# mryab/learning-at-home

Hardware: NVIDIA H100
Metric: DMoE training samples/sec (whole job, device-timed, max over ranks) (higher is better)
Workload: dtype bf16

## Files before the change

learning-at-home_b200/csrc/layernorm.cu:

```cuda
#include "sm90.cuh"
#include <cuda_fp8.h>
#include <stdlib.h>

#include <array>
#include <utility>

namespace lah {

constexpr float LN_EPS = 1e-5f;

constexpr int LN_MAX_C = 4096;

template <int C>
struct LnFwdCfg {
    static constexpr int NV = (C + 255) / 256;
    static constexpr bool TUNED = C >= 256 && (C & (C - 1)) == 0;
    static constexpr int R = TUNED ? ((NV * 4 <= 16) ? 4 : ((NV * 2 <= 16) ? 2 : 1)) : (NV <= 2 ? 4 : (NV <= 6 ? 2 : 1));
    static constexpr int MIN_BLOCKS = (TUNED || NV <= 12) ? 2 : 1;
};

static int ln_rows_per_warp(int dflt) {
    static int forced = -1;
    if (forced < 0) {
        const char* e = getenv("LAH_LN_ROWS");
        forced = e ? atoi(e) : 0;
    }
    return forced == 1 ? 1 : dflt;
}

template <int C, bool QUANT, int R>
__global__ void __launch_bounds__(256, LnFwdCfg<C>::MIN_BLOCKS) ln_relu_fwd_kernel(
    const bf16* __restrict__ h, bf16* __restrict__ a, float* __restrict__ mean_out, float* __restrict__ rstd_out,
    const float* __restrict__ gamma, const float* __restrict__ beta, const int* __restrict__ tile_group, int rows,
    int relu, uint8_t* __restrict__ aq, uint8_t* __restrict__ sf, int tile_shift) {
    constexpr int NV = LnFwdCfg<C>::NV;
    constexpr bool HALF = C % 256 != 0;
    static_assert(C % 128 == 0 && C <= LN_MAX_C && !(QUANT && HALF), "unsupported LayerNorm width");
    const int warp = threadIdx.x >> 5, lane = threadIdx.x & 31;
    const int row0 = (blockIdx.x * 8 + warp) * R;
    if (row0 >= rows) return;
    const int g = tile_group ? __ldg(tile_group + (row0 >> tile_shift)) : 0;
    if (g < 0) return;
    int4 q[R][NV];
#pragma unroll
    for (int r = 0; r < R; ++r) {
        const int4* hp = reinterpret_cast<const int4*>(h + static_cast<long long>(min(row0 + r, rows - 1)) * C);
#pragma unroll
        for (int j = 0; j < NV; ++j) {
            if constexpr (HALF) {
                if (j == NV - 1 && lane >= 16) {
                    q[r][j] = make_int4(0, 0, 0, 0);
                    continue;
                }
            }
            q[r][j] = ld_nc_v4(hp + j * 32 + lane);
        }
    }
    float mean[R], rstd[R];
#pragma unroll
    for (int r = 0; r < R; ++r) {
        float s = 0.f, ss = 0.f;
#pragma unroll
        for (int j = 0; j < NV; ++j) {
            const uint32_t w[4] = {(uint32_t)q[r][j].x, (uint32_t)q[r][j].y, (uint32_t)q[r][j].z, (uint32_t)q[r][j].w};
#pragma unroll
            for (int t = 0; t < 4; ++t) {
                const float2 f = unpack_bf16x2(w[t]);
                s += f.x + f.y;
                ss += f.x * f.x + f.y * f.y;
            }
        }
        s = warp_sum(s);
        ss = warp_sum(ss);
        mean[r] = s * (1.f / C);
        rstd[r] = rsqrtf(fmaxf(ss * (1.f / C) - mean[r] * mean[r], 0.f) + LN_EPS);
        if (lane == 0 && mean_out && row0 + r < rows) {
            mean_out[row0 + r] = mean[r];
            rstd_out[row0 + r] = rstd[r];
        }
    }
    const float* gp = gamma + static_cast<long long>(g) * C;
    const float* bp = beta + static_cast<long long>(g) * C;
#pragma unroll
    for (int j = 0; j < NV; ++j) {
        if constexpr (HALF) {
            if (j == NV - 1 && lane >= 16) break;
        }
        const int col = (j * 32 + lane) * 8;
        const int4 g0 = ld_nc_v4(reinterpret_cast<const int4*>(gp + col));
        const int4 g1 = ld_nc_v4(reinterpret_cast<const int4*>(gp + col + 4));
        const int4 b0 = ld_nc_v4(reinterpret_cast<const int4*>(bp + col));
        const int4 b1 = ld_nc_v4(reinterpret_cast<const int4*>(bp + col + 4));
        const float gg[8] = {__int_as_float(g0.x), __int_as_float(g0.y), __int_as_float(g0.z), __int_as_float(g0.w),
                             __int_as_float(g1.x), __int_as_float(g1.y), __int_as_float(g1.z), __int_as_float(g1.w)};
        const float bb[8] = {__int_as_float(b0.x), __int_as_float(b0.y), __int_as_float(b0.z), __int_as_float(b0.w),
                             __int_as_float(b1.x), __int_as_float(b1.y), __int_as_float(b1.z), __int_as_float(b1.w)};
#pragma unroll
        for (int r = 0; r < R; ++r) {
            const int row = row0 + r;
            if (row >= rows) continue;
            const uint32_t w[4] = {(uint32_t)q[r][j].x, (uint32_t)q[r][j].y, (uint32_t)q[r][j].z, (uint32_t)q[r][j].w};
            float y[8];
#pragma unroll
            for (int t = 0; t < 4; ++t) {
                const float2 f = unpack_bf16x2(w[t]);
                y[2 * t] = (f.x - mean[r]) * rstd[r] * gg[2 * t] + bb[2 * t];
                y[2 * t + 1] = (f.y - mean[r]) * rstd[r] * gg[2 * t + 1] + bb[2 * t + 1];
            }
            if (relu) {
#pragma unroll
                for (int t = 0; t < 8; ++t) y[t] = fmaxf(y[t], 0.f);
            }
            if (!QUANT || a) {
                int4 o;
                o.x = pack_bf16x2(y[0], y[1]);
                o.y = pack_bf16x2(y[2], y[3]);
                o.z = pack_bf16x2(y[4], y[5]);
                o.w = pack_bf16x2(y[6], y[7]);
                st_v4(reinterpret_cast<int4*>(a + static_cast<long long>(row) * C) + j * 32 + lane, o);
            }
            if (QUANT) {
                float amax = 0.f;
#pragma unroll
                for (int t = 0; t < 8; ++t) amax = fmaxf(amax, fabsf(y[t]));
                amax = fmaxf(amax, __shfl_xor_sync(0xffffffffu, amax, 1));
                amax = fmaxf(amax, __shfl_xor_sync(0xffffffffu, amax, 2));
                const uint32_t bits = __float_as_uint(amax * (1.f / 448.f));
                uint32_t e = ((bits >> 23) & 0xFFu) + ((bits & 0x7FFFFFu) ? 1u : 0u);
                e = min(max(e, 1u), 253u);
                const float inv = __uint_as_float((254u - e) << 23);
                uint2 o8;
                o8.x = static_cast<uint32_t>(__nv_cvt_float2_to_fp8x2(make_float2(y[0] * inv, y[1] * inv), __NV_SATFINITE, __NV_E4M3)) |
                       (static_cast<uint32_t>(__nv_cvt_float2_to_fp8x2(make_float2(y[2] * inv, y[3] * inv), __NV_SATFINITE, __NV_E4M3)) << 16);
                o8.y = static_cast<uint32_t>(__nv_cvt_float2_to_fp8x2(make_float2(y[4] * inv, y[5] * inv), __NV_SATFINITE, __NV_E4M3)) |
                       (static_cast<uint32_t>(__nv_cvt_float2_to_fp8x2(make_float2(y[6] * inv, y[7] * inv), __NV_SATFINITE, __NV_E4M3)) << 16);
                asm volatile("st.global.v2.u32 [%0], {%1, %2};" ::"l"(reinterpret_cast<uint2*>(aq + static_cast<long long>(row) * C) + j * 32 + lane),
                             "r"(o8.x), "r"(o8.y)
                             : "memory");
                if ((lane & 3) == 0) {
                    const int kb32 = j * 8 + (lane >> 2);
                    const int ra = row & 127;
                    const long long chunk = static_cast<long long>(row >> 7) * (C / 128) + (kb32 >> 2);
                    sf[chunk * 512 + ((ra & 31) * 4 + (ra >> 5)) * 4 + (kb32 & 3)] = static_cast<uint8_t>(e);
                }
            }
        }
    }
}

template <int C>
struct LnBwdCfg {
    static constexpr int THREADS = (C / 8 + 31) / 32 * 32;
    static constexpr int MIN_BLOCKS = (C <= 2048) ? 2 : 1;
    static constexpr int RB = ((THREADS / 32 * MIN_BLOCKS + 3) / 4 >= 4 && C != 2048) ? 2 : 4;
};

template <int C, bool RES>
__global__ void __launch_bounds__(LnBwdCfg<C>::THREADS, LnBwdCfg<C>::MIN_BLOCKS) ln_relu_bwd_kernel(const bf16* __restrict__ da, const bf16* __restrict__ h,
                                                            const float* __restrict__ mean_in,
                                                            const float* __restrict__ rstd_in,
                                                            const float* __restrict__ gamma,
                                                            const float* __restrict__ beta, bf16* __restrict__ dh,
                                                            float* __restrict__ part,
                                                            const int* __restrict__ tile_group, int rows, int relu, int tile_rows,
                                                            const bf16* __restrict__ dres) {
    constexpr int THREADS = LnBwdCfg<C>::THREADS;
    constexpr int WARPS = THREADS / 32;
    constexpr bool IDLE = THREADS * 8 != C;
    static_assert(C % 128 == 0 && C <= LN_MAX_C, "unsupported LayerNorm width");
    constexpr int RB = LnBwdCfg<C>::RB;
    __shared__ float red[WARPS][2 * RB];
    __shared__ float tot[2 * RB];
    const int tile = blockIdx.x;
    const int g = tile_group ? __ldg(tile_group + tile) : 0;
    if (g < 0) return;
    const int tid = threadIdx.x, warp = tid >> 5, lane = tid & 31;
    const int col = tid * 8;
    const bool live = !IDLE || col < C;
    float gam[8], bet[8];
    if (!live) {
#pragma unroll
        for (int t = 0; t < 8; ++t) gam[t] = bet[t] = 0.f;
    } else {
        const float* gp = gamma + static_cast<long long>(g) * C + col;
        const float* bp = beta + static_cast<long long>(g) * C + col;
        const float4 g0 = __ldg(reinterpret_cast<const float4*>(gp)), g1 = __ldg(reinterpret_cast<const float4*>(gp + 4));
        const float4 b0 = __ldg(reinterpret_cast<const float4*>(bp)), b1 = __ldg(reinterpret_cast<const float4*>(bp + 4));
        gam[0] = g0.x; gam[1] = g0.y; gam[2] = g0.z; gam[3] = g0.w; gam[4] = g1.x; gam[5] = g1.y; gam[6] = g1.z; gam[7] = g1.w;
        bet[0] = b0.x; bet[1] = b0.y; bet[2] = b0.z; bet[3] = b0.w; bet[4] = b1.x; bet[5] = b1.y; bet[6] = b1.z; bet[7] = b1.w;
    }
    float acc_dg[8], acc_db[8], acc_dbias[8];
#pragma unroll
    for (int t = 0; t < 8; ++t) acc_dg[t] = acc_db[t] = acc_dbias[t] = 0.f;

    const int row0 = tile * tile_rows;
    const int row_end = min(rows, row0 + tile_rows);
    int4 nqa[RB], nqh[RB];
    float nmu[RB], nrs[RB];
    auto issue_loads = [&](int rb) {
#pragma unroll
        for (int r = 0; r < RB; ++r) {
            const int row = rb + r;
            const int rr = row < row_end ? row : row0;
            const long long off = static_cast<long long>(rr) * C + col;
            if (live) {
                nqa[r] = ld_nc_v4(reinterpret_cast<const int4*>(da + off));
                nqh[r] = ld_nc_v4(reinterpret_cast<const int4*>(h + off));
            } else {
                nqa[r] = nqh[r] = make_int4(0, 0, 0, 0);
            }
            nmu[r] = __ldg(mean_in + rr);
            nrs[r] = __ldg(rstd_in + rr);
        }
    };
    issue_loads(row0);
    for (int rb = row0; rb < row_end; rb += RB) {
        float rs[RB];
        float part[2 * RB];
        int4 qa_c[RB], qh_c[RB];
        float mu_c[RB];
#pragma unroll
        for (int r = 0; r < RB; ++r) {
            qa_c[r] = nqa[r];
            qh_c[r] = nqh[r];
            mu_c[r] = nmu[r];
            rs[r] = nrs[r];
        }
        if (rb + RB < row_end) issue_loads(rb + RB);
        auto slice = [&](int r, bool ok, float (&gvv)[8], float (&xhh)[8]) {
            const uint32_t wa[4] = {(uint32_t)qa_c[r].x, (uint32_t)qa_c[r].y, (uint32_t)qa_c[r].z, (uint32_t)qa_c[r].w};
            const uint32_t wh[4] = {(uint32_t)qh_c[r].x, (uint32_t)qh_c[r].y, (uint32_t)qh_c[r].z, (uint32_t)qh_c[r].w};
#pragma unroll
            for (int t = 0; t < 4; ++t) {
                const float2 fa = unpack_bf16x2(wa[t]);
                const float2 fh = unpack_bf16x2(wh[t]);
                const float x0 = (fh.x - mu_c[r]) * rs[r], x1 = (fh.y - mu_c[r]) * rs[r];
                const float y0 = x0 * gam[2 * t] + bet[2 * t], y1 = x1 * gam[2 * t + 1] + bet[2 * t + 1];
                gvv[2 * t] = (ok && (!relu || y0 > 0.f)) ? fa.x : 0.f;
                gvv[2 * t + 1] = (ok && (!relu || y1 > 0.f)) ? fa.y : 0.f;
                xhh[2 * t] = x0;
                xhh[2 * t + 1] = x1;
            }
        };
#pragma unroll
        for (int r = 0; r < RB; ++r) {
            float gvv[8], xhh[8];
            slice(r, rb + r < row_end, gvv, xhh);
            float s1 = 0.f, s2 = 0.f;
#pragma unroll
            for (int t = 0; t < 8; ++t) {
                const float d = gvv[t] * gam[t];
                s1 += d;
                s2 += d * xhh[t];
            }
            part[2 * r] = s1;
            part[2 * r + 1] = s2;
        }
#pragma unroll
        for (int i = 0; i < 2 * RB; ++i) part[i] = warp_sum(part[i]);
        if (lane == 0) {
#pragma unroll
            for (int i = 0; i < 2 * RB; ++i) red[warp][i] = part[i];
        }
        __syncthreads();
        if (tid < 2 * RB) {
            float s = 0.f;
#pragma unroll
            for (int w = 0; w < WARPS; ++w) s += red[w][tid];
            tot[tid] = s * (1.f / C);
        }
        __syncthreads();
#pragma unroll
        for (int r = 0; r < RB; ++r) {
            const int row = rb + r;
            if (row >= row_end || !live) continue;
            float gvv[8], xhh[8];
            slice(r, true, gvv, xhh);
            const float m1 = tot[2 * r], m2 = tot[2 * r + 1];
            float o[8], res[8];
            if (RES) {
                const int4 qr = ld_nc_v4(reinterpret_cast<const int4*>(dres + static_cast<long long>(row) * C + col));
                const uint32_t wr[4] = {(uint32_t)qr.x, (uint32_t)qr.y, (uint32_t)qr.z, (uint32_t)qr.w};
#pragma unroll
                for (int t = 0; t < 4; ++t) {
                    const float2 fr = unpack_bf16x2(wr[t]);
                    res[2 * t] = fr.x;
                    res[2 * t + 1] = fr.y;
                }
            }
#pragma unroll
            for (int t = 0; t < 8; ++t) {
                o[t] = rs[r] * (gvv[t] * gam[t] - m1 - xhh[t] * m2);
                if (RES) o[t] += res[t];
                acc_db[t] += gvv[t];
                acc_dg[t] += gvv[t] * xhh[t];
                acc_dbias[t] += o[t];
            }
            int4 q;
            q.x = pack_bf16x2(o[0], o[1]);
            q.y = pack_bf16x2(o[2], o[3]);
            q.z = pack_bf16x2(o[4], o[5]);
            q.w = pack_bf16x2(o[6], o[7]);
            *reinterpret_cast<int4*>(dh + static_cast<long long>(row) * C + col) = q;
        }
    }
    if (!live) return;
    float* pg = part + static_cast<long long>(tile) * 3 * C + col;
#pragma unroll
    for (int t = 0; t < 8; ++t) {
        pg[t] = acc_dg[t];
        pg[C + t] = acc_db[t];
        pg[2 * C + t] = acc_dbias[t];
    }
}

__global__ void __launch_bounds__(512) grouped_colsum_kernel(const bf16* __restrict__ x, long long ldx,
                                                             float* __restrict__ part, int C,
                                                             const int* __restrict__ tile_group, int rows, int tile_rows) {
    __shared__ float2 sm[4][128];
    const int tile = blockIdx.x;
    const int g = tile_group ? __ldg(tile_group + tile) : 0;
    if (g < 0) return;
    const int cp = threadIdx.x & 127;
    const int phase = threadIdx.x >> 7;
    const int col = blockIdx.y * 256 + cp * 2;
    if (col >= C) return;
    const int row0 = tile * tile_rows, row_end = min(rows, row0 + tile_rows);
    float2 acc = make_float2(0.f, 0.f);
    for (int r = row0 + phase; r < row_end; r += 4) {
        const uint32_t u = __ldg(reinterpret_cast<const uint32_t*>(x + static_cast<long long>(r) * ldx + col));
        const float2 f = unpack_bf16x2(u);
        acc.x += f.x;
        acc.y += f.y;
    }
    sm[phase][cp] = acc;
    __syncthreads();
    if (phase == 0) {
        float2 s = sm[0][cp];
#pragma unroll
        for (int p = 1; p < 4; ++p) {
            s.x += sm[p][cp].x;
            s.y += sm[p][cp].y;
        }
        *reinterpret_cast<float2*>(part + static_cast<long long>(tile) * C + col) = s;
    }
}

__global__ void __launch_bounds__(256) group_tile_sum_kernel(const float* __restrict__ part, int num_tiles, int V, int C,
                                                             const int* __restrict__ tile_group, float* out0, float* out1,
                                                             float* out2) {
    const int i = blockIdx.x * blockDim.x + threadIdx.x;
    if (i >= V * C) return;
    const int v = i / C, c = i - v * C;
    float* out = v == 0 ? out0 : (v == 1 ? out1 : out2);
    int cur = -1;
    float acc = 0.f;
    for (int t = 0; t < num_tiles; ++t) {
        const int g = tile_group ? __ldg(tile_group + t) : 0;
        if (g < 0) continue;
        if (g != cur) {
            if (cur >= 0) out[static_cast<long long>(cur) * C + c] += acc;
            cur = g;
            acc = 0.f;
        }
        acc += __ldg(part + (static_cast<long long>(t) * V + v) * C + c);
    }
    if (cur >= 0) out[static_cast<long long>(cur) * C + c] += acc;
}

using LnFwdLaunch = void (*)(const void*, void*, float*, float*, const float*, const float*, const int*, int, int, int,
                             cudaStream_t);
using LnBwdLaunch = void (*)(const void*, const void*, const float*, const float*, const float*, const float*, void*,
                             float*, float*, float*, float*, const int*, int, int, int, const void*, cudaStream_t);

template <int C>
void ln_fwd_launch(const void* h, void* a, float* mean, float* rstd, const float* gamma, const float* beta,
                   const int* tile_group, int rows, int relu, int tile_shift, cudaStream_t st) {
    constexpr int RR = LnFwdCfg<C>::R;
    if constexpr (LnFwdCfg<C>::TUNED) {
        if (ln_rows_per_warp(RR) == 1) {
            ln_relu_fwd_kernel<C, false, 1><<<(rows + 7) / 8, 256, 0, st>>>(
                (const bf16*)h, (bf16*)a, mean, rstd, gamma, beta, tile_group, rows, relu, nullptr, nullptr, tile_shift);
            return;
        }
    }
    ln_relu_fwd_kernel<C, false, RR><<<(rows + 8 * RR - 1) / (8 * RR), 256, 0, st>>>(
        (const bf16*)h, (bf16*)a, mean, rstd, gamma, beta, tile_group, rows, relu, nullptr, nullptr, tile_shift);
}

template <int C>
void ln_bwd_launch(const void* da, const void* h, const float* mean, const float* rstd, const float* gamma,
                   const float* beta, void* dh, float* dgamma, float* dbeta, float* dbias, float* part,
                   const int* tile_group, int rows, int relu, int tile_rows, const void* dres, cudaStream_t st) {
    const int grid = (rows + tile_rows - 1) / tile_rows;
    constexpr int T = LnBwdCfg<C>::THREADS;
    if (dres)
        ln_relu_bwd_kernel<C, true><<<grid, T, 0, st>>>((const bf16*)da, (const bf16*)h, mean, rstd, gamma, beta,
                                                        (bf16*)dh, part, tile_group, rows, relu, tile_rows,
                                                        (const bf16*)dres);
    else
        ln_relu_bwd_kernel<C, false><<<grid, T, 0, st>>>((const bf16*)da, (const bf16*)h, mean, rstd, gamma, beta,
                                                         (bf16*)dh, part, tile_group, rows, relu, tile_rows, nullptr);
    group_tile_sum_kernel<<<(3 * C + 255) / 256, 256, 0, st>>>(part, grid, 3, C, tile_group, dgamma, dbeta, dbias);
}

template <int... I>
constexpr auto ln_fwd_table(std::integer_sequence<int, I...>) {
    return std::array<LnFwdLaunch, sizeof...(I)>{ln_fwd_launch<(I + 1) * 128>...};
}
template <int... I>
constexpr auto ln_bwd_table(std::integer_sequence<int, I...>) {
    return std::array<LnBwdLaunch, sizeof...(I)>{ln_bwd_launch<(I + 1) * 128>...};
}
constexpr auto kLnFwd = ln_fwd_table(std::make_integer_sequence<int, LN_MAX_C / 128>{});
constexpr auto kLnBwd = ln_bwd_table(std::make_integer_sequence<int, LN_MAX_C / 128>{});

static bool ln_width_ok(int C) { return C > 0 && C % 128 == 0 && C <= LN_MAX_C; }

}

using namespace lah;

extern "C" {

static int shift_of(int tile_rows) {
    int s = 0;
    while ((1 << s) < tile_rows) ++s;
    return ((1 << s) == tile_rows && tile_rows >= 8) ? s : -1;
}

int lah_ln_relu_fwd(const void* h, void* a, float* mean, float* rstd, const float* gamma, const float* beta,
                    const int* tile_group, int rows, int C, int relu, int tile_rows, cudaStream_t st) {
    if (rows <= 0) return 0;
    const int tile_shift = shift_of(tile_rows);
    if (tile_shift < 0 || !ln_width_ok(C)) return -2;
    kLnFwd[C / 128 - 1](h, a, mean, rstd, gamma, beta, tile_group, rows, relu, tile_shift, st);
    return -(int)cudaGetLastError();
}

int lah_ln_relu_fwd_q(const void* h, void* a, float* mean, float* rstd, const float* gamma, const float* beta,
                      const int* tile_group, int rows, int C, int relu, void* aq, void* sf, cudaStream_t st) {
    if (rows <= 0) return 0;
#define LAH_LN_FWD(CC)                                                                                          \
    if (C == CC) {                                                                                              \
        constexpr int RR = LnFwdCfg<CC>::R;                                                                     \
        if (ln_rows_per_warp(RR) == 1)                                                                          \
            ln_relu_fwd_kernel<CC, true, 1><<<(rows + 7) / 8, 256, 0, st>>>(                                  \
                (const bf16*)h, (bf16*)a, mean, rstd, gamma, beta, tile_group, rows, relu, (uint8_t*)aq, (uint8_t*)sf, 7);   \
        else                                                                                                    \
            ln_relu_fwd_kernel<CC, true, RR><<<(rows + 8 * RR - 1) / (8 * RR), 256, 0, st>>>(                 \
                (const bf16*)h, (bf16*)a, mean, rstd, gamma, beta, tile_group, rows, relu, (uint8_t*)aq, (uint8_t*)sf, 7);   \
        return -(int)cudaGetLastError();                                                                        \
    }
    LAH_LN_FWD(256) LAH_LN_FWD(512) LAH_LN_FWD(1024) LAH_LN_FWD(2048) LAH_LN_FWD(4096)
#undef LAH_LN_FWD
    return -2;
}

int lah_ln_relu_bwd(const void* da, const void* h, const float* mean, const float* rstd, const float* gamma,
                    const float* beta, void* dh, float* dgamma, float* dbeta, float* dbias, float* part,
                    const int* tile_group, int rows, int C, int relu, int tile_rows, const void* dres, cudaStream_t st) {
    if (rows <= 0) return 0;
    if (shift_of(tile_rows) < 0 || !ln_width_ok(C)) return -2;
    kLnBwd[C / 128 - 1](da, h, mean, rstd, gamma, beta, dh, dgamma, dbeta, dbias, part, tile_group, rows, relu,
                        tile_rows, dres, st);
    return -(int)cudaGetLastError();
}

int lah_grouped_colsum(const void* x, long long ldx, float* out, float* part, int C, const int* tile_group, int rows,
                       int tile_rows, cudaStream_t st) {
    if (rows <= 0) return 0;
    if (C % 128 || shift_of(tile_rows) < 0) return -2;
    const int tiles = (rows + tile_rows - 1) / tile_rows;
    dim3 grid(tiles, (C + 255) / 256);
    grouped_colsum_kernel<<<grid, 512, 0, st>>>((const bf16*)x, ldx, part, C, tile_group, rows, tile_rows);
    group_tile_sum_kernel<<<(C + 255) / 256, 256, 0, st>>>(part, tiles, 1, C, tile_group, out, nullptr, nullptr);
    return -(int)cudaGetLastError();
}

}
```

learning-at-home_b200/csrc/small_m.cu:

```cuda
#include "sm90.cuh"
#include <climits>

namespace lah {
namespace smallm {

constexpr int BM = 128;
constexpr int BK = 64;
constexpr int MMA_K = 16;
constexpr int BN_MAX = 128;
constexpr int NUM_THREADS = 288;

namespace sab {

constexpr int STAGES = 6;
constexpr int A_BYTES = BM * BK * 2;
constexpr int B_BYTES = BN_MAX * BK * 2;
constexpr int STAGE_BYTES = A_BYTES + B_BYTES;
constexpr int BAR_OFFSET = STAGES * STAGE_BYTES;
constexpr int QD = 4;
constexpr int MAX_G = 1023;
constexpr int CUM_OFFSET = BAR_OFFSET + (2 * STAGES + 2 * QD) * 8 + QD * 4 + 16;
constexpr int SMEM_TOTAL = CUM_OFFSET + (MAX_G + 1) * 4 + 1024;
static_assert(SMEM_TOTAL <= 232448, "shared memory budget");

struct Params {
    int G, M_out, K;
    const int* group_off;
    const int* group_rows;
    bf16* out;
    long long ldo;
    const float* bias;
    const bf16* residual;
    long long ldr;
    const int* wait_flags;
    int wait_count, wait_epoch;
    const int* epoch_base;
    int* status;
    int* tile_counter;
};

__device__ __forceinline__ int box_rows_of(int nn) { return nn <= 16 ? 16 : (nn <= 32 ? 32 : (nn <= 64 ? 64 : 128)); }

__device__ __forceinline__ int find_group(const int* cum, int G, int gc) {
    int lo = 0, hi = G - 1;
    while (lo < hi) {
        const int mid = (lo + hi + 1) >> 1;
        if (cum[mid] <= gc) lo = mid; else hi = mid - 1;
    }
    return lo;
}

template <int NB, bool A_MN>
__device__ __forceinline__ void sab_tile(const Params& p, uint8_t* smem, uint64_t* full_bar, uint64_t* empty_bar, int& stage,
                                         uint32_t& phase, int num_kb, int wg, int warp, int lane, int g, int ms, int row0,
                                         int nn) {
    float acc[NB / 2];
    constexpr uint32_t A_KSTEP = A_MN ? MMA_K * 128 : MMA_K * 2;
    int prev_stage = -1;
    for (int kb = 0; kb < num_kb; ++kb) {
        mbar_wait(&full_bar[stage], phase);
        const uint32_t sa = smem_u32(smem + stage * STAGE_BYTES) + wg * (A_MN ? BK * 128 : 64 * 128);
        const uint32_t sb = smem_u32(smem + stage * STAGE_BYTES + A_BYTES);
        wgmma_fence();
#pragma unroll
        for (int k = 0; k < BK / MMA_K; ++k) {
            const uint64_t da = make_smem_desc_sw128(sa + k * A_KSTEP, BK * 128, 1024);
            const uint64_t db = make_smem_desc_sw128(sb + k * (MMA_K * 2), 0, 1024);
            const uint32_t accum = (kb > 0 || k > 0) ? 1u : 0u;
            if constexpr (NB == 16) wgmma_bf16_n16<A_MN, 0>(acc, da, db, accum);
            if constexpr (NB == 32) wgmma_bf16_n32<A_MN, 0>(acc, da, db, accum);
            if constexpr (NB == 64) wgmma_bf16_n64<A_MN, 0>(acc, da, db, accum);
            if constexpr (NB == 128) wgmma_bf16_n128<A_MN, 0>(acc, da, db, accum);
        }
        wgmma_commit();
        wgmma_wait<1>();
        if (prev_stage >= 0) {
            __syncwarp();
            if (lane == 0) mbar_arrive(&empty_bar[prev_stage]);
        }
        prev_stage = stage;
        if (++stage == STAGES) {
            stage = 0;
            phase ^= 1;
        }
    }
    wgmma_wait<0>();
    wgmma_fence_regs(acc);
    __syncwarp();
    if (lane == 0 && prev_stage >= 0) mbar_arrive(&empty_bar[prev_stage]);

    const int n16 = (nn + 15) & ~15;
#pragma unroll
    for (int h = 0; h < 2; ++h) {
        const int feat = ms * BM + wg * 64 + (warp & 3) * 16 + (lane >> 2) + 8 * h;
        const float bias = p.bias ? __ldg(p.bias + static_cast<long long>(g) * p.M_out + feat) : 0.f;
#pragma unroll
        for (int j = 0; j < NB / 8; ++j) {
#pragma unroll
            for (int e = 0; e < 2; ++e) {
                const int n = 8 * j + 2 * (lane & 3) + e;
                if (n < n16) {
                    const long long row = row0 + n;
                    float v = acc[4 * j + 2 * h + e] + bias;
                    if (p.residual) v += __bfloat162float(p.residual[row * p.ldr + feat]);
                    p.out[row * p.ldo + feat] = __float2bfloat16(v);
                }
            }
        }
    }
}

template <bool A_MN>
__global__ void __launch_bounds__(NUM_THREADS, 1)
swapab_kernel(const Params p, const __grid_constant__ CUtensorMap tmA, const __grid_constant__ CUtensorMap tmB16,
              const __grid_constant__ CUtensorMap tmB32, const __grid_constant__ CUtensorMap tmB64,
              const __grid_constant__ CUtensorMap tmB128) {
    extern __shared__ uint8_t smem_raw[];
    uint8_t* smem = reinterpret_cast<uint8_t*>((reinterpret_cast<uintptr_t>(smem_raw) + 1023) & ~uintptr_t(1023));
    uint64_t* full_bar = reinterpret_cast<uint64_t*>(smem + BAR_OFFSET);
    uint64_t* empty_bar = full_bar + STAGES;
    uint64_t* q_full = empty_bar + STAGES;
    uint64_t* q_empty = q_full + QD;
    volatile int* q_tile = reinterpret_cast<volatile int*>(q_empty + QD);
    int* cum = reinterpret_cast<int*>(smem + CUM_OFFSET);

    const int warp = threadIdx.x >> 5;
    const int lane = threadIdx.x & 31;

    if (warp == 0) {
        int carry = 0;
        for (int base = 0; base < p.G; base += 32) {
            const int g = base + lane;
            int x = g < p.G ? (__ldg(p.group_rows + g) + BN_MAX - 1) / BN_MAX : 0;
#pragma unroll
            for (int d = 1; d < 32; d <<= 1) {
                const int y = __shfl_up_sync(0xffffffffu, x, d);
                if (lane >= d) x += y;
            }
            if (g < p.G) cum[g + 1] = carry + x;
            carry += __shfl_sync(0xffffffffu, x, 31);
        }
        if (lane == 0) cum[0] = 0;
    }
    if (warp == 8 && lane == 0) {
        tma_prefetch_desc(&tmA);
        tma_prefetch_desc(&tmB16);
        tma_prefetch_desc(&tmB32);
        tma_prefetch_desc(&tmB64);
        tma_prefetch_desc(&tmB128);
        for (int i = 0; i < STAGES; ++i) {
            mbar_init(&full_bar[i], 1);
            mbar_init(&empty_bar[i], 8);
        }
        for (int i = 0; i < QD; ++i) {
            mbar_init(&q_full[i], 1);
            mbar_init(&q_empty[i], 8);
        }
        fence_mbar_init();
    }
    __syncthreads();

    const int m_slices = p.M_out / BM;
    const int total = cum[p.G] * m_slices;
    const int num_kb = p.K / BK;

    if (warp == 8) {
        if (lane != 0) return;
        if (p.wait_flags) {
            const int epoch = p.wait_epoch + (p.epoch_base ? *p.epoch_base : 0);
            const unsigned long long t_wait = globaltimer_ns();
            for (int sidx = 0; sidx < p.wait_count; ++sidx)
                spin_flag_ft(p.wait_flags + sidx, epoch, p.status, sidx, p.epoch_base ? p.epoch_base[1] : 0);
            if (blockIdx.x == 0) atomicAdd(reinterpret_cast<unsigned long long*>(p.status + 2), globaltimer_ns() - t_wait);
            fence_proxy_async_global();
        }
        int stage = 0, qi = 0;
        uint32_t phase = 0, qphase = 0;
        while (true) {
            const int tile = atomicAdd(p.tile_counter, 1);
            mbar_wait(&q_empty[qi], qphase ^ 1);
            q_tile[qi] = tile;
            mbar_arrive(&q_full[qi]);
            if (++qi == QD) {
                qi = 0;
                qphase ^= 1;
            }
            if (tile >= total) break;
            const int gc = tile / m_slices, ms = tile - gc * m_slices;
            const int g = find_group(cum, p.G, gc);
            const int n0 = (gc - cum[g]) * BN_MAX;
            const int rows = __ldg(p.group_rows + g);
            const int off = __ldg(p.group_off + g);
            const int box = box_rows_of(min(rows - n0, BN_MAX));
            const CUtensorMap* tmB = box == 16 ? &tmB16 : (box == 32 ? &tmB32 : (box == 64 ? &tmB64 : &tmB128));
            for (int kb = 0; kb < num_kb; ++kb) {
                mbar_wait(&empty_bar[stage], phase ^ 1);
                uint8_t* sa = smem + stage * STAGE_BYTES;
                uint8_t* sb = sa + A_BYTES;
                const int k = kb * BK;
                mbar_arrive_expect_tx(&full_bar[stage], A_BYTES + box * 128);
                if (!A_MN) {
                    tma_load_3d(sa, &tmA, &full_bar[stage], k, ms * BM, g);
                } else {
#pragma unroll
                    for (int i = 0; i < BM / 64; ++i)
                        tma_load_3d(sa + i * (BK * 128), &tmA, &full_bar[stage], ms * BM + i * 64, k, g);
                }
                tma_load_2d(sb, tmB, &full_bar[stage], k, off + n0);
                if (++stage == STAGES) {
                    stage = 0;
                    phase ^= 1;
                }
            }
        }
        return;
    }

    const int wg = warp >> 2;
    int stage = 0, qi = 0;
    uint32_t phase = 0, qphase = 0;
    while (true) {
        mbar_wait(&q_full[qi], qphase);
        const int tile = q_tile[qi];
        __syncwarp();
        if (lane == 0) mbar_arrive(&q_empty[qi]);
        if (++qi == QD) {
            qi = 0;
            qphase ^= 1;
        }
        if (tile >= total) break;
        const int gc = tile / m_slices, ms = tile - gc * m_slices;
        const int g = find_group(cum, p.G, gc);
        const int n0 = (gc - cum[g]) * BN_MAX;
        const int nn = min(__ldg(p.group_rows + g) - n0, BN_MAX);
        const int row0 = __ldg(p.group_off + g) + n0;
        switch (box_rows_of(nn)) {
            case 16: sab_tile<16, A_MN>(p, smem, full_bar, empty_bar, stage, phase, num_kb, wg, warp, lane, g, ms, row0, nn); break;
            case 32: sab_tile<32, A_MN>(p, smem, full_bar, empty_bar, stage, phase, num_kb, wg, warp, lane, g, ms, row0, nn); break;
            case 64: sab_tile<64, A_MN>(p, smem, full_bar, empty_bar, stage, phase, num_kb, wg, warp, lane, g, ms, row0, nn); break;
            default: sab_tile<128, A_MN>(p, smem, full_bar, empty_bar, stage, phase, num_kb, wg, warp, lane, g, ms, row0, nn); break;
        }
    }
}

}

namespace wa {

constexpr int WBK = 32;
constexpr int OP_STAGES = 2;
constexpr int OP_STAGE_BYTES = 2 * (WBK * BM * 2);
constexpr int OP_BYTES = OP_STAGES * OP_STAGE_BYTES;
constexpr int BAND_ROWS = 4;
constexpr int CHUNKS = 16 / BAND_ROWS;
constexpr int SUB_COLS = 32;
constexpr int SUB_BYTES = BM / CHUNKS * SUB_COLS * 4;
constexpr int ARR_BYTES = (BN_MAX / SUB_COLS) * SUB_BYTES;
constexpr int ST_STAGES = 3;
constexpr int ST_STAGE_BYTES = 4 * ARR_BYTES;
constexpr int ST_OFFSET = OP_BYTES;
constexpr int BAR_OFFSET = ST_OFFSET + ST_STAGES * ST_STAGE_BYTES;
constexpr int QD = 4;
constexpr int SMEM_TOTAL = BAR_OFFSET + (2 * OP_STAGES + 2 * ST_STAGES + 2 * QD) * 8 + QD * 4 + 16 + 1024;
static_assert(ST_STAGES <= CHUNKS, "the producer issues a tile's first ST_STAGES chunks before its remaining k-blocks");
static_assert(OP_STAGE_BYTES % 1024 == 0 && SUB_BYTES % 1024 == 0, "128-B swizzle atoms need 1 KB alignment");
static_assert(SMEM_TOTAL <= 232448, "shared memory budget");

struct Params {
    int G, N, K;
    const int* group_off;
    const int* group_rows;
    const int* skip;
    const int* step;
    float* p;
    float* m;
    float* v;
    float* vmax;
    bf16* p_bf16;
    float lr, beta1, beta2, eps;
    int amsgrad;
    float wd;
    int* tile_counter;
    const int* poison;
};

constexpr int WD_NONE = 0, WD_L2 = 1, WD_DECOUPLED = 2;

struct Tile {
    int g, mt, nt;
};

struct StateMaps {
    CUtensorMap a[4];
};

__device__ __forceinline__ void state_chunk_tma(const StateMaps& tm, int n_arr, uint8_t* ss, uint64_t* bar, int col0, int srow,
                                                int c) {
    for (int a = 0; a < n_arr; ++a)
#pragma unroll
        for (int q = 0; q < BN_MAX / SUB_COLS; ++q) {
            uint8_t* s = ss + a * ARR_BYTES + q * SUB_BYTES;
            if (bar) tma_load_3d(s, &tm.a[a], bar, col0 + q * SUB_COLS, BAND_ROWS * c, srow / 16);
            else tma_store_3d(&tm.a[a], s, col0 + q * SUB_COLS, BAND_ROWS * c, srow / 16);
        }
}

template <int WD>
__global__ void __launch_bounds__(NUM_THREADS, 1)
wgrad_adam_kernel(const Params p, const __grid_constant__ CUtensorMap tmDY, const __grid_constant__ CUtensorMap tmX,
                  const __grid_constant__ StateMaps tmS) {
    extern __shared__ uint8_t smem_raw[];
    uint8_t* smem = reinterpret_cast<uint8_t*>((reinterpret_cast<uintptr_t>(smem_raw) + 1023) & ~uintptr_t(1023));
    uint8_t* st_smem = smem + ST_OFFSET;
    uint64_t* op_full = reinterpret_cast<uint64_t*>(smem + BAR_OFFSET);
    uint64_t* op_empty = op_full + OP_STAGES;
    uint64_t* st_full = op_empty + OP_STAGES;
    uint64_t* st_empty = st_full + ST_STAGES;
    uint64_t* q_full = st_empty + ST_STAGES;
    uint64_t* q_empty = q_full + QD;
    volatile int* q_tile = reinterpret_cast<volatile int*>(q_empty + QD);

    const int warp = threadIdx.x >> 5;
    const int lane = threadIdx.x & 31;
    if (p.poison && (*p.poison & 1)) return;
    const int n_arr = p.amsgrad ? 4 : 3;

    if (warp == 8 && lane == 0) {
        tma_prefetch_desc(&tmDY);
        tma_prefetch_desc(&tmX);
        for (int a = 0; a < n_arr; ++a) tma_prefetch_desc(&tmS.a[a]);
        for (int i = 0; i < OP_STAGES; ++i) {
            mbar_init(&op_full[i], 1);
            mbar_init(&op_empty[i], 8);
        }
        for (int i = 0; i < ST_STAGES; ++i) {
            mbar_init(&st_full[i], 1);
            mbar_init(&st_empty[i], 1);
        }
        for (int i = 0; i < QD; ++i) {
            mbar_init(&q_full[i], 1);
            mbar_init(&q_empty[i], 8);
        }
        fence_mbar_init();
    }
    __syncthreads();

    const int n_tiles = p.K / BN_MAX;
    const int tiles_per_group = (p.N / BM) * n_tiles;
    const int total = p.G * tiles_per_group;
    auto decode = [&](int tile) {
        Tile t;
        t.g = tile / tiles_per_group;
        const int r = tile - t.g * tiles_per_group;
        t.mt = r / n_tiles;
        t.nt = r - t.mt * n_tiles;
        return t;
    };

    if (warp == 8) {
        if (lane != 0) return;
        uint32_t phase = 0, qphase = 0, sphase = 0;
        int qi = 0, stage = 0, sstage = 0;
        while (true) {
            int tile;
            while (true) {
                tile = atomicAdd(p.tile_counter, 1);
                if (tile >= total) break;
                const int g = tile / tiles_per_group;
                if (__ldg(p.group_rows + g) > 0 && !(p.skip && __ldg(p.skip + 2 * g) >= 0)) break;
                atomicMax(p.tile_counter, (g + 1) * tiles_per_group);
            }
            mbar_wait(&q_empty[qi], qphase ^ 1);
            q_tile[qi] = tile;
            mbar_arrive(&q_full[qi]);
            if (++qi == QD) {
                qi = 0;
                qphase ^= 1;
            }
            if (tile >= total) break;
            const Tile t = decode(tile);
            const int off = __ldg(p.group_off + t.g), rows = __ldg(p.group_rows + t.g);
            const int srow = t.g * p.N + t.mt * BM;
            auto load_chunk = [&](int c) {
                mbar_wait(&st_empty[sstage], sphase ^ 1);
                mbar_arrive_expect_tx(&st_full[sstage], n_arr * ARR_BYTES);
                state_chunk_tma(tmS, n_arr, st_smem + sstage * ST_STAGE_BYTES, &st_full[sstage], t.nt * BN_MAX, srow, c);
                if (++sstage == ST_STAGES) {
                    sstage = 0;
                    sphase ^= 1;
                }
            };
            for (int t0 = 0; t0 < rows; t0 += WBK) {
                mbar_wait(&op_empty[stage], phase ^ 1);
                mbar_arrive_expect_tx(&op_full[stage], OP_STAGE_BYTES);
                uint8_t* sa = smem + stage * OP_STAGE_BYTES;
                uint8_t* sb = sa + WBK * BM * 2;
#pragma unroll
                for (int i = 0; i < BM / 64; ++i)
                    tma_load_2d(sa + i * (WBK * 128), &tmDY, &op_full[stage], t.mt * BM + i * 64, off + t0);
#pragma unroll
                for (int i = 0; i < BN_MAX / 64; ++i)
                    tma_load_2d(sb + i * (WBK * 128), &tmX, &op_full[stage], t.nt * BN_MAX + i * 64, off + t0);
                if (++stage == OP_STAGES) {
                    stage = 0;
                    phase ^= 1;
                }
                if (t0 == 0)
                    for (int c = 0; c < ST_STAGES; ++c) load_chunk(c);
            }
            for (int c = ST_STAGES; c < CHUNKS; ++c) load_chunk(c);
        }
        return;
    }

    const int wg = warp >> 2;
    int qi = 0, stage = 0, sstage = 0;
    uint32_t phase = 0, qphase = 0, sphase = 0;
    float acc[BN_MAX / 2];
    float xg[BN_MAX / 8];
    const int lrow = wg * 64 + (warp & 3) * 16 + (lane >> 2);
    const int brow = (lane >> 2) & 3;
    const int R = warp * BAND_ROWS + brow;
    const int jflip = 2 * (brow & 1);
    while (true) {
        mbar_wait(&q_full[qi], qphase);
        const int tile = q_tile[qi];
        __syncwarp();
        if (lane == 0) mbar_arrive(&q_empty[qi]);
        if (++qi == QD) {
            qi = 0;
            qphase ^= 1;
        }
        if (tile >= total) break;
        const Tile t = decode(tile);
        const int rows = __ldg(p.group_rows + t.g);
        int prev_stage = -1;
        for (int t0 = 0; t0 < rows; t0 += WBK) {
            mbar_wait(&op_full[stage], phase);
            const uint32_t sa = smem_u32(smem + stage * OP_STAGE_BYTES) + wg * (WBK * 128);
            const uint32_t sb = smem_u32(smem + stage * OP_STAGE_BYTES + WBK * BM * 2);
            const int ksteps = min(WBK / MMA_K, (rows - t0 + MMA_K - 1) / MMA_K);
            wgmma_fence();
            for (int k = 0; k < ksteps; ++k) {
                const uint64_t da = make_smem_desc_sw128(sa + k * (MMA_K * 128), WBK * 128, 1024);
                const uint64_t db = make_smem_desc_sw128(sb + k * (MMA_K * 128), WBK * 128, 1024);
                wgmma_bf16_n128<1, 1>(acc, da, db, (t0 > 0 || k > 0) ? 1u : 0u);
            }
            wgmma_commit();
            wgmma_wait<1>();
            if (prev_stage >= 0) {
                __syncwarp();
                if (lane == 0) mbar_arrive(&op_empty[prev_stage]);
            }
            prev_stage = stage;
            if (++stage == OP_STAGES) {
                stage = 0;
                phase ^= 1;
            }
        }
        wgmma_wait<0>();
        wgmma_fence_regs(acc);
        __syncwarp();
        if (lane == 0 && prev_stage >= 0) mbar_arrive(&op_empty[prev_stage]);

        const float st = static_cast<float>(__ldg(p.step + t.g));
        const float step_size = p.lr / (1.f - powf(p.beta1, st));
        const float inv_sqrt_bc2 = rsqrtf(1.f - powf(p.beta2, st));
        const int srow = t.g * p.N + t.mt * BM;
        const int col_base = t.nt * BN_MAX + 2 * (lane & 3);
#pragma unroll
        for (int c = 0; c < CHUNKS; ++c) {
            mbar_wait(&st_full[sstage], sphase);
            uint8_t* ss = st_smem + sstage * ST_STAGE_BYTES;
            if ((c & 1) == 0) {
#pragma unroll
                for (int i = 0; i < BN_MAX / 8; ++i) xg[i] = __shfl_xor_sync(0xffffffffu, acc[4 * (BN_MAX / 16 + i / 2) + i % 2], 16);
            }
            const bool own = (lane >> 4) == (c & 1);
            const long long o_row = (static_cast<long long>(srow) + (own ? lrow : lrow ^ 4) + 8 * (c >> 1)) * p.K + col_base;
            const int jbase = own ? 0 : BN_MAX / 16;
#pragma unroll
            for (int k = 0; k < BN_MAX / 16; ++k) {
                const int j = jbase + (k ^ jflip);
                const int so = (j >> 2) * SUB_BYTES + R * 128 + (((2 * (j & 3) + ((lane & 3) >> 1)) ^ (R & 7)) << 4) +
                               8 * (lane & 1);
                float2* sp = reinterpret_cast<float2*>(ss + so);
                float2* sm = reinterpret_cast<float2*>(ss + ARR_BYTES + so);
                float2* sv = reinterpret_cast<float2*>(ss + 2 * ARR_BYTES + so);
                float2* svm = reinterpret_cast<float2*>(ss + 3 * ARR_BYTES + so);
                float2 pw = *sp, m = *sm, v = *sv;
                float2 vm = p.amsgrad ? *svm : make_float2(0.f, 0.f);
                float* pp = &pw.x; float* mp = &m.x; float* vp = &v.x; float* vmp = &vm.x;
#pragma unroll
                for (int e = 0; e < 2; ++e) {
                    float grad = own ? (jflip ? acc[4 * (k ^ 2) + e] : acc[4 * k + e])
                                     : (jflip ? xg[2 * (k ^ 2) + e] : xg[2 * k + e]);
                    if constexpr (WD == WD_L2) grad += p.wd * pp[e];
                    if constexpr (WD == WD_DECOUPLED) pp[e] = __fmul_rn(pp[e], p.wd);
                    mp[e] = mp[e] + (1.f - p.beta1) * (grad - mp[e]);
                    vp[e] = vp[e] * p.beta2 + (1.f - p.beta2) * grad * grad;
                    float denom;
                    if (p.amsgrad) {
                        vmp[e] = fmaxf(vmp[e], vp[e]);
                        denom = sqrtf(vmp[e]) * inv_sqrt_bc2 + p.eps;
                    } else {
                        denom = sqrtf(vp[e]) * inv_sqrt_bc2 + p.eps;
                    }
                    pp[e] -= step_size * (mp[e] / denom);
                }
                *sp = pw;
                *sm = m;
                *sv = v;
                if (p.amsgrad) *svm = vm;
                *reinterpret_cast<uint32_t*>(p.p_bf16 + o_row + 8 * j) = pack_bf16x2(pw.x, pw.y);
            }
            fence_proxy_async_smem();
            named_bar_sync(1, 256);
            if (threadIdx.x == 0) {
                state_chunk_tma(tmS, n_arr, ss, nullptr, t.nt * BN_MAX, srow, c);
                tma_store_commit();
                tma_store_wait_read<0>();
                mbar_arrive(&st_empty[sstage]);
            }
            if (++sstage == ST_STAGES) {
                sstage = 0;
                sphase ^= 1;
            }
            if (c == 1) {
#pragma unroll
                for (int j = 0; j < BN_MAX / 8; ++j) {
                    acc[4 * j] = acc[4 * j + 2];
                    acc[4 * j + 1] = acc[4 * j + 3];
                }
            }
        }
    }
    if (threadIdx.x == 0) tma_store_wait<0>();
}

}
}
}

using namespace lah;
using namespace lah::smallm;

extern "C" const int* lah_get_epoch_base();

static int* tile_counter() {
    static int* ctr = nullptr;
    if (!ctr) {
        if (cudaMalloc(&ctr, 256) != cudaSuccess) return nullptr;
        cudaMemset(ctr, 0, 256);
    }
    return ctr;
}
static const int* g_poison = nullptr;

extern "C" {

int lah_set_poison_word(const int* status) {
    g_poison = status;
    return 0;
}
const int* lah_get_poison_word() { return g_poison; }

int lah_swapab_linear(const void* x, long long ldx, int x_rows, const void* W, int G, int M_out, int K, int a_mn,
                      void* out, long long ldo, const int* group_off, const int* group_rows, const float* bias,
                      const void* residual, long long ldr, const int* wait_flags, int wait_count, int wait_epoch,
                      const int* epoch_base, int* status, int max_ctas, cudaStream_t st) {
    if ((K % BK) || (M_out % BM) || (ldx % 8) || G > sab::MAX_G) return -2;
    CUtensorMap tmA, tmB[4];
    if (!a_mn) {
        uint64_t dims[3] = {(uint64_t)K, (uint64_t)M_out, (uint64_t)G};
        uint64_t str[2] = {(uint64_t)K * 2, (uint64_t)M_out * K * 2};
        uint32_t box[3] = {BK, BM, 1};
        int r = make_tmap(&tmA, CU_TENSOR_MAP_DATA_TYPE_BFLOAT16, 3, W, dims, str, box);
        if (r) return r;
    } else {
        uint64_t dims[3] = {(uint64_t)M_out, (uint64_t)K, (uint64_t)G};
        uint64_t str[2] = {(uint64_t)M_out * 2, (uint64_t)M_out * K * 2};
        uint32_t box[3] = {64, BK, 1};
        int r = make_tmap(&tmA, CU_TENSOR_MAP_DATA_TYPE_BFLOAT16, 3, W, dims, str, box);
        if (r) return r;
    }
    const uint32_t boxes[4] = {16, 32, 64, 128};
    for (int i = 0; i < 4; ++i) {
        uint64_t dims[2] = {(uint64_t)K, (uint64_t)x_rows};
        uint64_t str[1] = {(uint64_t)ldx * 2};
        uint32_t box[2] = {BK, boxes[i]};
        int r = make_tmap(&tmB[i], CU_TENSOR_MAP_DATA_TYPE_BFLOAT16, 2, x, dims, str, box);
        if (r) return r;
    }
    sab::Params p;
    p.G = G; p.M_out = M_out; p.K = K; p.group_off = group_off; p.group_rows = group_rows; p.out = (bf16*)out; p.ldo = ldo;
    p.bias = bias; p.residual = (const bf16*)residual; p.ldr = ldr; p.wait_flags = wait_flags; p.wait_count = wait_count;
    p.wait_epoch = wait_epoch; p.epoch_base = epoch_base ? epoch_base : lah_get_epoch_base(); p.status = status;
    p.tile_counter = tile_counter();
    if (!p.tile_counter) return -3;
    const long long total = 1ll * (M_out / BM) * (G + x_rows / BN_MAX);
    if (total <= 0 || G <= 0) return 0;
    if (cudaMemsetAsync(p.tile_counter, 0, sizeof(int), st) != cudaSuccess) return -4;
    const int ctas = persistent_grid(total, max_ctas);
    if (!a_mn) {
        if (int e = set_max_dynamic_smem<sab::swapab_kernel<false>>(sab::SMEM_TOTAL)) return e;
        sab::swapab_kernel<false><<<ctas, NUM_THREADS, sab::SMEM_TOTAL, st>>>(p, tmA, tmB[0], tmB[1], tmB[2], tmB[3]);
    } else {
        if (int e = set_max_dynamic_smem<sab::swapab_kernel<true>>(sab::SMEM_TOTAL)) return e;
        sab::swapab_kernel<true><<<ctas, NUM_THREADS, sab::SMEM_TOTAL, st>>>(p, tmA, tmB[0], tmB[1], tmB[2], tmB[3]);
    }
    return -(int)cudaGetLastError();
}

int lah_wgrad_adam_wd(const void* dy, long long lddy, const void* x, long long ldx, int total_rows, int G, int N, int K,
                      const int* group_off, const int* group_rows, const int* skip, const int* step, float* p, float* m,
                      float* v, float* vmax, void* p_bf16, float lr, float beta1, float beta2, float eps, int amsgrad,
                      float weight_decay, float decay, int max_ctas, cudaStream_t st) {
    if ((N % BM) || (K % BN_MAX) || (lddy % 8) || (ldx % 8) || 1ll * G * N > INT_MAX) return -2;
    if (decay != 1.f && weight_decay != 0.f) return -2;
    if (amsgrad && !vmax) return -2;
    CUtensorMap tmDY, tmX;
    wa::StateMaps tmS;
    {
        float* arrs[4] = {p, m, v, amsgrad ? vmax : p};
        uint64_t dims[3] = {(uint64_t)K, 16, (uint64_t)G * N / 16};
        uint64_t str[2] = {(uint64_t)K * 4, (uint64_t)K * 64};
        uint32_t box[3] = {wa::SUB_COLS, wa::BAND_ROWS, BM / 16};
        for (int a = 0; a < 4; ++a) {
            int r = make_tmap(&tmS.a[a], CU_TENSOR_MAP_DATA_TYPE_FLOAT32, 3, arrs[a], dims, str, box);
            if (r) return r;
        }
    }
    {
        uint64_t dims[2] = {(uint64_t)N, (uint64_t)total_rows};
        uint64_t str[1] = {(uint64_t)lddy * 2};
        uint32_t box[2] = {64, wa::WBK};
        int r = make_tmap(&tmDY, CU_TENSOR_MAP_DATA_TYPE_BFLOAT16, 2, dy, dims, str, box);
        if (r) return r;
    }
    {
        uint64_t dims[2] = {(uint64_t)K, (uint64_t)total_rows};
        uint64_t str[1] = {(uint64_t)ldx * 2};
        uint32_t box[2] = {64, wa::WBK};
        int r = make_tmap(&tmX, CU_TENSOR_MAP_DATA_TYPE_BFLOAT16, 2, x, dims, str, box);
        if (r) return r;
    }
    wa::Params a;
    a.G = G; a.N = N; a.K = K; a.group_off = group_off; a.group_rows = group_rows; a.skip = skip; a.step = step;
    a.p = p; a.m = m; a.v = v; a.vmax = vmax; a.p_bf16 = (bf16*)p_bf16; a.lr = lr; a.beta1 = beta1; a.beta2 = beta2; a.eps = eps; a.amsgrad = amsgrad;
    a.wd = decay != 1.f ? decay : weight_decay;
    a.tile_counter = tile_counter() ? tile_counter() + 16 : nullptr;
    a.poison = g_poison;
    if (!a.tile_counter) return -3;
    const long long total = 1ll * G * (N / BM) * (K / BN_MAX);
    if (total <= 0) return 0;
    if (cudaMemsetAsync(a.tile_counter, 0, sizeof(int), st) != cudaSuccess) return -4;
    const int ctas = persistent_grid(total, max_ctas);
    if (decay != 1.f) {
        if (int e = set_max_dynamic_smem<wa::wgrad_adam_kernel<wa::WD_DECOUPLED>>(wa::SMEM_TOTAL)) return e;
        wa::wgrad_adam_kernel<wa::WD_DECOUPLED><<<ctas, NUM_THREADS, wa::SMEM_TOTAL, st>>>(a, tmDY, tmX, tmS);
    } else if (weight_decay != 0.f) {
        if (int e = set_max_dynamic_smem<wa::wgrad_adam_kernel<wa::WD_L2>>(wa::SMEM_TOTAL)) return e;
        wa::wgrad_adam_kernel<wa::WD_L2><<<ctas, NUM_THREADS, wa::SMEM_TOTAL, st>>>(a, tmDY, tmX, tmS);
    } else {
        if (int e = set_max_dynamic_smem<wa::wgrad_adam_kernel<wa::WD_NONE>>(wa::SMEM_TOTAL)) return e;
        wa::wgrad_adam_kernel<wa::WD_NONE><<<ctas, NUM_THREADS, wa::SMEM_TOTAL, st>>>(a, tmDY, tmX, tmS);
    }
    return -(int)cudaGetLastError();
}

int lah_wgrad_adam(const void* dy, long long lddy, const void* x, long long ldx, int total_rows, int G, int N, int K,
                   const int* group_off, const int* group_rows, const int* skip, const int* step, float* p, float* m,
                   float* v, float* vmax, void* p_bf16, float lr, float beta1, float beta2, float eps, int amsgrad,
                   int max_ctas, cudaStream_t st) {
    return lah_wgrad_adam_wd(dy, lddy, x, ldx, total_rows, G, N, K, group_off, group_rows, skip, step, p, m, v, vmax, p_bf16,
                             lr, beta1, beta2, eps, amsgrad, 0.f, 1.f, max_ctas, st);
}

}
```

Before: 12890.

## Self-reset tile counter in swap-AB kernel; batch loads in group tile sum

The persistent swap-AB GEMM no longer clears its dynamic tile counter with a memset before each launch. Instead the last CTA's producer resets the counter, using a second arrival counter, so one memset node per call drops off the stream. The group tile-sum kernel now preloads 16 tiles of group ids and partials into registers before reducing, which exposes memory-level parallelism. It also switches its flushes to atomicAdd, which adds atomic cost and depends on the in-kernel reset being correctly ordered with the next launch.

```diff
diff --git a/learning-at-home_b200/csrc/layernorm.cu b/learning-at-home_b200/csrc/layernorm.cu
--- a/learning-at-home_b200/csrc/layernorm.cu
+++ b/learning-at-home_b200/csrc/layernorm.cu
@@ -346,6 +346,7 @@
     }
 }
 
+constexpr int TILE_BATCH = 16;
 __global__ void __launch_bounds__(256) group_tile_sum_kernel(const float* __restrict__ part, int num_tiles, int V, int C,
                                                              const int* __restrict__ tile_group, float* out0, float* out1,
                                                              float* out2) {
@@ -355,17 +356,28 @@
     float* out = v == 0 ? out0 : (v == 1 ? out1 : out2);
     int cur = -1;
     float acc = 0.f;
-    for (int t = 0; t < num_tiles; ++t) {
-        const int g = tile_group ? __ldg(tile_group + t) : 0;
-        if (g < 0) continue;
-        if (g != cur) {
-            if (cur >= 0) out[static_cast<long long>(cur) * C + c] += acc;
-            cur = g;
-            acc = 0.f;
-        }
-        acc += __ldg(part + (static_cast<long long>(t) * V + v) * C + c);
-    }
-    if (cur >= 0) out[static_cast<long long>(cur) * C + c] += acc;
+    for (int t0 = 0; t0 < num_tiles; t0 += TILE_BATCH) {
+        int gs[TILE_BATCH];
+        float ps[TILE_BATCH];
+#pragma unroll
+        for (int j = 0; j < TILE_BATCH; ++j) {
+            const int t = t0 + j;
+            gs[j] = t < num_tiles ? (tile_group ? __ldg(tile_group + t) : 0) : -1;
+            ps[j] = t < num_tiles ? __ldg(part + (static_cast<long long>(t) * V + v) * C + c) : 0.f;
+        }
+#pragma unroll
+        for (int j = 0; j < TILE_BATCH; ++j) {
+            const int g = gs[j];
+            if (g < 0) continue;
+            if (g != cur) {
+                if (cur >= 0) atomicAdd(out + static_cast<long long>(cur) * C + c, acc);
+                cur = g;
+                acc = 0.f;
+            }
+            acc += ps[j];
+        }
+    }
+    if (cur >= 0) atomicAdd(out + static_cast<long long>(cur) * C + c, acc);
 }
 
 using LnFwdLaunch = void (*)(const void*, void*, float*, float*, const float*, const float*, const int*, int, int, int,
diff --git a/learning-at-home_b200/csrc/small_m.cu b/learning-at-home_b200/csrc/small_m.cu
--- a/learning-at-home_b200/csrc/small_m.cu
+++ b/learning-at-home_b200/csrc/small_m.cu
@@ -212,6 +212,11 @@
                     phase ^= 1;
                 }
             }
+        }
+        __threadfence();
+        if (atomicAdd(p.tile_counter + 1, 1) == static_cast<int>(gridDim.x) - 1) {
+            atomicExch(p.tile_counter, 0);
+            atomicExch(p.tile_counter + 1, 0);
         }
         return;
     }
@@ -551,7 +556,7 @@
     static int* ctr = nullptr;
     if (!ctr) {
         if (cudaMalloc(&ctr, 256) != cudaSuccess) return nullptr;
-        cudaMemset(ctr, 0, 256);
+        if (cudaMemset(ctr, 0, 256) != cudaSuccess || cudaDeviceSynchronize() != cudaSuccess) return nullptr;
     }
     return ctr;
 }
@@ -600,7 +605,6 @@
     if (!p.tile_counter) return -3;
     const long long total = 1ll * (M_out / BM) * (G + x_rows / BN_MAX);
     if (total <= 0 || G <= 0) return 0;
-    if (cudaMemsetAsync(p.tile_counter, 0, sizeof(int), st) != cudaSuccess) return -4;
     const int ctas = persistent_grid(total, max_ctas);
     if (!a_mn) {
         if (int e = set_max_dynamic_smem<sab::swapab_kernel<false>>(sab::SMEM_TOTAL)) return e;
```

After: 12930, median of 6. No clear change (+0.3%).
